# facebook/zstd

Hardware: NVIDIA H100
Metric: compress GB/s (input) at level 1 (higher is better)
Workload: dtype u8

## Files before the change

zstd_b200/csrc/zb_bitpack.cuh:

```cuda
#ifndef ZB_BITPACK_CUH
#define ZB_BITPACK_CUH
#include "zb_device.cuh"

struct ZbdParW { u32* words; u64 acc; u32 nacc; u32 widx; u32 first; };

__device__ __forceinline__ void zbd_pw_init(ZbdParW* w, u32* words, u64 bitPos)
{
    w->words = words; w->acc = 0; w->nacc = (u32)(bitPos & 31u); w->widx = (u32)(bitPos >> 5); w->first = 1;
}
__device__ __forceinline__ void zbd_pw_add(ZbdParW* w, u32 value, u32 nbBits)
{
    w->acc |= (u64)value << w->nacc;
    w->nacc += nbBits;
    if (w->nacc >= 32u) {
        u32 const lo = (u32)w->acc;
        if (w->first) { if (lo) atomicOr(&w->words[w->widx], lo); w->first = 0; }
        else w->words[w->widx] = lo;
        w->widx++;
        w->acc >>= 32;
        w->nacc -= 32u;
    }
}
__device__ __forceinline__ void zbd_pw_finish(ZbdParW* w)
{
    u32 const lo = (u32)w->acc;
    if (w->nacc && lo) atomicOr(&w->words[w->widx], lo);
}

#endif
```

zstd_b200/csrc/zb_entropy.cuh:

```cuda
#ifndef ZB_ENTROPY_CUH
#define ZB_ENTROPY_CUH
#include "zb_device.cuh"

#define ZBD_ERR 0xFFFFFFFFu

struct ZbdBitW { u8* out; u32 pos; u64 acc; u32 nacc; };
__device__ __forceinline__ void zbd_bw_init(ZbdBitW* w, u8* out) { w->out = out; w->pos = 0; w->acc = 0; w->nacc = 0; }
__device__ __forceinline__ void zbd_bw_add(ZbdBitW* w, u32 value, u32 nbBits)
{
    if (!nbBits) return;
    w->acc |= (u64)(value & ((1u << nbBits) - 1u)) << w->nacc;
    w->nacc += nbBits;
    while (w->nacc >= 8) { w->out[w->pos++] = (u8)w->acc; w->acc >>= 8; w->nacc -= 8; }
}
__device__ __forceinline__ u32 zbd_bw_close(ZbdBitW* w)
{
    zbd_bw_add(w, 1, 1);
    if (w->nacc) w->out[w->pos++] = (u8)w->acc;
    return w->pos;
}


__device__ __forceinline__ u32 zbd_fse_optimalTableLog(u32 maxTableLog, u32 srcSize, u32 maxSymbolValue, u32 minus)
{
    u32 const fromSource = zb_hb32(srcSize - 1u) - minus;
    u32 const needSrc = zb_hb32(srcSize) + 1u, needAlphabet = zb_hb32(maxSymbolValue) + 2u;
    u32 const floorLog = needSrc < needAlphabet ? needSrc : needAlphabet;
// ... 154 lines not shown

__device__ __forceinline__ u32 zbd_fse_initState2(const ZbdFseCTable* ct, u32 symbol)
{
    u32 const dnb = ct->deltaNbBits[symbol];
    u32 const nbBitsOut = (dnb + (1u << 15)) >> 16;
    u32 const value = (nbBitsOut << 16) - dnb;
    return ct->nextState[(int)(value >> nbBitsOut) + ct->deltaFindState[symbol]];
}
__device__ __forceinline__ u32 zbd_fse_step(const ZbdFseCTable* ct, u32 state, u32 symbol, u32* bits, u32* nb)
{
    u32 const nbBitsOut = (state + ct->deltaNbBits[symbol]) >> 16;
    *nb = nbBitsOut;
    *bits = state & ((1u << nbBitsOut) - 1u);
    return ct->nextState[(int)(state >> nbBitsOut) + ct->deltaFindState[symbol]];
}

struct ZbdHufWksp {
    u32 A[256];
    u16 rankSym[256];
    u8  len[256];
    u8  weights[256];
    u32 nl[16];
    u32 firstCode[16];
    u32 wcount[16];
    short wnorm[16];
    u8  symAt[64];
    u16 cum[66];
    u32 maxLen, nz;
    ZbdFseCTable wct;
};

template <int HUF_THREADS>
__device__ inline u32 zbc_huf_build(ZbdHufWksp* w, const u32* count, u32 maxSymbolValue, u32 target, u32* enc)
{
    u32 const tid = threadIdx.x;
    if (tid == 0) w->nz = 0;
    __syncthreads();
    {   u32 mine = 0;
        for (u32 s = tid; s < 256u; s += HUF_THREADS) {
            u32 const c = s <= maxSymbolValue ? count[s] : 0u;
            w->len[s] = 0;
            if (c) {
                u32 r = 0;
                for (u32 j = 0; j <= maxSymbolValue; j++) { u32 const cj = count[j]; r += (cj > c || (cj == c && j < s)) ? 1u : 0u; }
                w->rankSym[r] = (u16)s;
                mine++;
            }
        }
        if (mine) atomicAdd(&w->nz, mine);
    }
    __syncthreads();
    u32 const nz = w->nz;
    for (u32 i = tid; i < nz; i += HUF_THREADS) w->A[i] = count[w->rankSym[nz - 1u - i]];
    __syncthreads();
    if (tid == 0) {
        u32* const A = w->A;
        u32 root = 0, leaf = 2, next;
        A[0] += A[1];
        for (next = 1; next + 1u < nz; next++) {
            if (leaf >= nz || A[root] < A[leaf]) { A[next] = A[root]; A[root++] = next; } else A[next] = A[leaf++];
            if (leaf >= nz || (root < next && A[root] < A[leaf])) { A[next] += A[root]; A[root++] = next; } else A[next] += A[leaf++];
        }
        A[nz - 2u] = 0;
        for (next = nz - 2u; next-- > 0u; ) A[next] = A[A[next]] + 1u;
        {   int avbl = 1, used = 0, depth = 0;
            int rt = (int)nz - 2, nx = (int)nz - 1;
            while (avbl > 0) {
                while (rt >= 0 && (int)A[rt] == depth) { used++; rt--; }
                while (avbl > used) { A[nx--] = (u32)depth; avbl--; }
                avbl = 2 * used; depth++; used = 0;
            }
        }
        for (u32 l = 0; l < 16u; l++) w->nl[l] = 0;
    }
    __syncthreads();
    u32 const deepest = w->A[0];
// ... 6 lines not shown
            u32 K = 0;
            for (u32 l = target + 1u; l < 16u; l++) { nl[target] += nl[l]; nl[l] = 0; }
            for (u32 l = 1; l <= target; l++) K += nl[l] << (target - l);
            for (u32 E = K - (1u << target); E > 0u; E--) {
                u32 b = target - 1u;
                while (nl[b] == 0u) b--;
                nl[b]--; nl[b + 1u] += 2u; nl[target]--;
            }
            maxLen = target;
        }
        while (nl[maxLen] == 0u) maxLen--;
        w->maxLen = maxLen;
        u32 v = 0;
        for (u32 l = maxLen; l > 0u; l--) { w->firstCode[l] = v; v = (v + nl[l]) >> 1; }
    }
    __syncthreads();
    u32 const maxLen = w->maxLen;
    for (u32 r = tid; r < nz; r += HUF_THREADS) {
        u32 l = 1, acc = w->nl[1];
        while (r >= acc) { l++; acc += w->nl[l]; }
        w->len[w->rankSym[r]] = (u8)l;
    }
    __syncthreads();
    for (u32 s = tid; s < 256u; s += HUF_THREADS) {
        u32 const l = w->len[s];
        u32 e = 0;
        if (l) {
            u32 idx = 0;
            for (u32 j = 0; j < s; j++) idx += (w->len[j] == l) ? 1u : 0u;
            e = (w->firstCode[l] + idx) | (l << 16);
        }
        enc[s] = e;
    }
    __syncthreads();
    return maxLen;
}

template <int HUF_THREADS>
__device__ inline u32 zbc_huf_writeHeader(ZbdHufWksp* w, u8* dst, const u32* enc, u32 maxSymbolValue, u32 huffLog, u32* sh_result)
{
    u32 const tid = threadIdx.x, lane = tid & 31u;
    u8* const wt = w->weights;
    u32 const wtSize = maxSymbolValue;
    if (tid < 16u) w->wcount[tid] = 0;
    __syncthreads();
    for (u32 n = tid; n < wtSize; n += HUF_THREADS) {
        u32 const nb = enc[n] >> 16;
        u32 const v = nb ? huffLog + 1u - nb : 0u;
        wt[n] = (u8)v;
        atomicAdd(&w->wcount[v], 1u);
    }
    if (tid == 0) wt[wtSize] = 0;
    __syncthreads();
    if (tid < 32u) {
        u32 hSize = 0;
// ... 59 lines not shown
```

zstd_b200/csrc/zb_literals.cu:

```cuda
#include "zb_entropy.cuh"
#include "zb_kernels.h"

#define LIT_THREADS 128
#ifndef LIT_MIN_CTAS
#define LIT_MIN_CTAS 12
#endif
#define LIT_WARPS (LIT_THREADS / 32)
#define LIT_WIN 256u

__device__ void zb_hist256(const u8* __restrict__ src, u32 n, u32 (*whist)[256], u32* count)
{
    u32 const tid = threadIdx.x, warp = tid >> 5, lane = tid & 31u;
    for (u32 i = tid; i < LIT_WARPS * 256; i += LIT_THREADS) (&whist[0][0])[i] = 0;
    __syncthreads();
    u32 const head = (u32)((uintptr_t)src & 15u);
    const uint4* const v4 = reinterpret_cast<const uint4*>(src - head);
    u32 const seg = (n + 3u) / 4u;
    u32 const beg = min(warp * seg, n) + head, end = min((warp + 1u) * seg, n) + head;
    if (beg < end) {
        u32 const vLo = beg >> 4, nVec = ((end - 1u) >> 4) - vLo + 1u;
        uint4 nx = lane < nVec ? __ldg(v4 + vLo + lane) : make_uint4(0, 0, 0, 0);
        for (u32 i = lane; i < nVec; i += 32u) {
            uint4 const q = nx;
            if (i + 32u < nVec) nx = __ldg(v4 + vLo + i + 32u);
            u32 const p0 = (vLo + i) << 4;
            u32 const kLo = beg > p0 ? beg - p0 : 0u, kHi = min(end - p0, 16u);
            u32 const w[4] = { q.x, q.y, q.z, q.w };
#pragma unroll
            for (u32 k = 0; k < 16u; k++)
                if (k >= kLo && k < kHi) atomicAdd(&whist[warp][(w[k >> 2] >> (8u * (k & 3u))) & 0xFFu], 1u);
        }
    }
    __syncthreads();
    for (u32 sym = tid; sym < 256u; sym += LIT_THREADS) {
        u32 s = 0;
#pragma unroll
        for (int w = 0; w < LIT_WARPS; w++) s += whist[w][sym];
        count[sym] = s;
    }
    __syncthreads();
}

__device__ void zb_hist_stats(const u32* count, u32* red, u32* largestOut, u32* maxSymOut)
{
    u32 const tid = threadIdx.x;
    u32 c = 0, key = 0;
    for (u32 sym = tid; sym < 256u; sym += LIT_THREADS) { u32 const v = count[sym]; c = max(c, v); key = max(key, v ? sym : 0u); }
#pragma unroll
    for (int o = 16; o > 0; o >>= 1) {
        c = max(c, __shfl_xor_sync(ZB_FULL, c, o));
        key = max(key, __shfl_xor_sync(ZB_FULL, key, o));
    }
    if ((tid & 31) == 0) { red[tid >> 5] = c; red[8 + (tid >> 5)] = key; }
    __syncthreads();
    if (tid == 0) {
        u32 l = 0, m = 0;
        for (int w = 0; w < LIT_WARPS; w++) { l = max(l, red[w]); m = max(m, red[8 + w]); }
        *largestOut = l; *maxSymOut = m;
    }
    __syncthreads();
}

__device__ __forceinline__ void zb_huf_stream(const u8* __restrict__ lit, u32 beg, u32 end, const u32* enc, u32* win, u32* ow,
                                              u32 bitPos, u32 lane)
{
    const uint4* const v4 = reinterpret_cast<const uint4*>(lit);
    uint4 const zero = make_uint4(0, 0, 0, 0);
    u32 const vHi = (end - 1u) >> 4, nVec = vHi - (beg >> 4) + 1u;
    u32 const firstW = bitPos >> 5;
    uint4 q1 = lane < nVec ? __ldg(v4 + vHi - lane) : zero;
    uint4 q2 = lane + 32u < nVec ? __ldg(v4 + vHi - lane - 32u) : zero;
    for (u32 t = 0; t < nVec; t += 32u) {
        uint4 const q = q1;
        q1 = q2;
        q2 = t + 64u + lane < nVec ? __ldg(v4 + vHi - (t + 64u + lane)) : zero;
        u32 kLo = 0, kHi = 0;
        if (t + lane < nVec) { u32 const p0 = (vHi - t - lane) << 4; kLo = beg > p0 ? beg - p0 : 0u; kHi = min(end - p0, 16u); }
        u32 const w[4] = { q.x, q.y, q.z, q.w };
        u32 nb = 0;
#pragma unroll
        for (u32 k = 0; k < 16u; k++) {
            u32 const e = enc[(w[k >> 2] >> (8u * (k & 3u))) & 0xFFu];
            nb += (k >= kLo && k < kHi) ? e >> 16 : 0u;
        }
        u32 incl = nb;
#pragma unroll
        for (u32 o = 1; o < 32u; o <<= 1) { u32 const x = __shfl_up_sync(ZB_FULL, incl, o); if (lane >= o) incl += x; }
        u32 const tileBits = __shfl_sync(ZB_FULL, incl, 31);
        {
            u32 const p = bitPos + incl - nb;
            u32 widx = p >> 5, nacc = p & 31u, first = 1;
            u64 acc = 0;
#pragma unroll
            for (int k = 15; k >= 0; k--) {
                u32 const e = ((u32)k >= kLo && (u32)k < kHi) ? enc[(w[k >> 2] >> (8u * (k & 3u))) & 0xFFu] : 0u;
                acc |= (u64)(e & 0xFFFFu) << nacc;
                nacc += e >> 16;
                if (k & 1) continue;
                bool const full = nacc >= 32u;
                u32* const wp = win + widx % LIT_WIN;
                if (full && first == 0u) *wp = (u32)acc;
                if (full && first != 0u) atomicOr(wp, (u32)acc);
                first = full ? 0u : first;
                widx += full ? 1u : 0u;
                acc = full ? (acc >> 32) : acc;
                nacc -= full ? 32u : 0u;
            }
            if (nacc != 0u && (u32)acc != 0u) atomicOr(win + widx % LIT_WIN, (u32)acc);
        }
        __syncwarp();
        u32 const wEnd = (bitPos + tileBits) >> 5;
        for (u32 k = (bitPos >> 5) + lane; k < wEnd; k += 32u) {
            u32 const v = win[k % LIT_WIN];
            win[k % LIT_WIN] = 0u;
            if (k == firstW) atomicOr(ow + k, v); else ow[k] = v;
        }
        __syncwarp();
        bitPos += tileBits;
    }
    if (lane == 0) atomicOr(ow + (bitPos >> 5), win[(bitPos >> 5) % LIT_WIN] | (1u << (bitPos & 31u)));
}

__global__ void __launch_bounds__(LIT_THREADS, LIT_MIN_CTAS)
zb_literals_kernel(const ZbBlock* __restrict__ blocks, ZbParams prm, ZbStrides sd, const ZbDictEntropy* __restrict__ de,
                   const u8* __restrict__ lits, u8* __restrict__ body, ZbBlockMeta* __restrict__ meta)
{
    __shared__ __align__(16) u32 whist[LIT_WARPS][256];
    __shared__ ZbdHufWksp wk;
    __shared__ u32 count[256];
    __shared__ u32 enc[256];
    __shared__ __align__(16) u8 hdr[288];
    __shared__ u32 red[16];
    __shared__ u32 sh_largest, sh_maxSym, sh_mode, sh_hSize, sh_usePrev;
    __shared__ u32 sh_bits[LIT_WARPS];

    u32 const tid = threadIdx.x, warp = tid >> 5, lane = tid & 31u;
    u32 const b = blockIdx.x;
    ZbBlockMeta const m = meta[b];
    if (m.forceRaw) return;
    u32 const n = m.litSize;
    const u8* const lit = lits + (size_t)b * sd.lit;
    u8* const out = body + (size_t)b * sd.body;
    enum { MODE_RAW = 0, MODE_RLE = 1, MODE_HUF = 2 };

    u32 repeat = (de != nullptr && (blocks[b].flags & ZB_FLAG_FIRST) && de->present) ? de->hufRepeat : 0u;
    bool const preferRepeat = (n <= 1024u);
    u32 const lhSize = 3u + (n >= 1024u) + (n >= 16384u);
    u32 const nbStreams = (n < 256u || (repeat == 2u && lhSize == 3u)) ? 1u : 4u;
    u32 mode = MODE_HUF;
    bool usePrev = false;
    if (prm.litDisabled || n < (repeat == 2u ? 6u : 64u)) mode = MODE_RAW;
    if (mode == MODE_HUF && preferRepeat && repeat == 2u) usePrev = true;
    if (mode == MODE_HUF && !usePrev) {
        bool const suspect = (m.nbSeq == 0) || (n / m.nbSeq >= 20u);
        if (suspect && n >= 4096u * 10u) {
            u32 l1, l2;
            zb_hist256(lit, 4096u, whist, count);
            zb_hist_stats(count, red, &sh_largest, &sh_maxSym);
            l1 = sh_largest;
            __syncthreads();
            zb_hist256(lit + n - 4096u, 4096u, whist, count);
            zb_hist_stats(count, red, &sh_largest, &sh_maxSym);
            l2 = sh_largest;
            __syncthreads();
            if (l1 + l2 <= ((2u * 4096u) >> 7) + 4u) mode = MODE_RAW;
        }
    }
    if (mode == MODE_HUF) zb_hist256(lit, n, whist, count);
    if (mode == MODE_HUF && !usePrev) {
        zb_hist_stats(count, red, &sh_largest, &sh_maxSym);
        u32 const largest = sh_largest;
        if (largest == n) mode = MODE_RLE;
        else if (largest <= (n >> 7) + 4u) mode = MODE_RAW;
    }
    if (mode == MODE_HUF && !usePrev && repeat == 1u) {
        int bad = 0;
        for (u32 sym = tid; sym < 256u; sym += LIT_THREADS) bad |= (sym <= sh_maxSym) && count[sym] != 0u && (de->hufEnc[sym] >> 16) == 0u;
        if (__syncthreads_or(bad) || de->hufMaxSymbol < sh_maxSym) repeat = 0u;
    }
    if (mode == MODE_HUF && !usePrev && preferRepeat && repeat != 0u) usePrev = true;
    if (mode == MODE_HUF && !usePrev) {
        u32 const maxSym = sh_maxSym;
        u32 const huffLog = zbd_fse_optimalTableLog(11, n, maxSym, 1);
        u32 const maxBits = zbc_huf_build<LIT_THREADS>(&wk, count, maxSym, huffLog, enc);
        u32 const hSizeNew = (maxBits == ZBD_ERR) ? ZBD_ERR : zbc_huf_writeHeader<LIT_THREADS>(&wk, hdr, enc, maxSym, maxBits, &sh_hSize);
        if (tid == 0) {
            u32 md = MODE_HUF, hSize = 0, prev = 0;
            if (hSizeNew == ZBD_ERR) md = MODE_RAW;
            else {
                hSize = hSizeNew;
                if (repeat != 0u) {
                    u32 oldBits = 0, newBits = 0;
                    for (u32 sy = 0; sy <= maxSym; sy++) { oldBits += (de->hufEnc[sy] >> 16) * count[sy]; newBits += (enc[sy] >> 16) * count[sy]; }
                    if ((oldBits >> 3) <= hSize + (newBits >> 3) || hSize + 12u >= n) prev = 1;
                }
                if (!prev && hSize + 12u >= n) md = MODE_RAW;
            }
            sh_mode = md; sh_hSize = hSize; sh_usePrev = prev;
        }
        __syncthreads();
        mode = sh_mode;
        usePrev = sh_usePrev != 0u;
    }
    if (mode == MODE_HUF && usePrev) {
        __syncthreads();
        for (u32 sym = tid; sym < 256u; sym += LIT_THREADS) enc[sym] = de->hufEnc[sym];
        if (tid == 0) sh_hSize = 0;
        __syncthreads();
    }

    u32 const hType = usePrev ? 3u : 2u;
    u32 const seg = (n + 3u) / 4u;
    u32 streamSize[4] = { 0u, 0u, 0u, 0u };
    u32 hSize = 0, total = 0;
    if (mode == MODE_HUF) {
        hSize = sh_hSize;
        u32 bits = 0;
        for (u32 sym = lane; sym < 256u; sym += 32u) bits += whist[warp][sym] * (enc[sym] >> 16);
#pragma unroll
        for (int o = 16; o > 0; o >>= 1) bits += __shfl_xor_sync(ZB_FULL, bits, o);
        if (lane == 0) sh_bits[warp] = bits;
        __syncthreads();
        if (nbStreams == 4u) for (u32 k = 0; k < 4u; k++) streamSize[k] = (sh_bits[k] + 1u + 7u) >> 3;
        else streamSize[0] = (sh_bits[0] + sh_bits[1] + sh_bits[2] + sh_bits[3] + 1u + 7u) >> 3;
        u32 cSize = 0; bool tooBig = false;
#pragma unroll
        for (u32 k = 0; k < 4u; k++) { cSize += streamSize[k]; tooBig |= (streamSize[k] > 65535u); }
        if (nbStreams == 4u) cSize += 6u;
        total = hSize + cSize;
        if (nbStreams == 4u && tooBig) mode = MODE_RAW;
        else if (total >= n - 1u) mode = MODE_RAW;
        else if (total >= n - ((n >> 6) + 2u)) mode = MODE_RAW;
        else if (total == 1u) {
            int diff = 0;
            if (n < 8u) for (u32 i = tid; i < n; i += LIT_THREADS) diff |= (lit[i] != lit[0]);
            if (!__syncthreads_or(diff)) mode = MODE_RLE;
        }
    }

    if (mode == MODE_RAW) {
        u32 const flSize = 1u + (n > 31u) + (n > 4095u);
        if (tid == 0) {
            if (flSize == 1) out[0] = (u8)(0u + (n << 3));
            else if (flSize == 2) { u32 const v = 0u + (1u << 2) + (n << 4); out[0] = (u8)v; out[1] = (u8)(v >> 8); }
            else { u32 const v = 0u + (3u << 2) + (n << 4); out[0] = (u8)v; out[1] = (u8)(v >> 8); out[2] = (u8)(v >> 16); }
            meta[b].litSecSize = flSize + n;
        }
        for (u32 i = tid; i < n; i += LIT_THREADS) out[flSize + i] = lit[i];
        return;
    }
    if (mode == MODE_RLE) {
        if (tid == 0) {
            u32 const flSize = 1u + (n > 31u) + (n > 4095u);
            if (flSize == 1) out[0] = (u8)(1u + (n << 3));
            else if (flSize == 2) { u32 const v = 1u + (1u << 2) + (n << 4); out[0] = (u8)v; out[1] = (u8)(v >> 8); }
            else { u32 const v = 1u + (3u << 2) + (n << 4); out[0] = (u8)v; out[1] = (u8)(v >> 8); out[2] = (u8)(v >> 16); }
            out[flSize] = lit[0];
            meta[b].litSecSize = flSize + 1u;
        }
        return;
    }

    u32 sOff = lhSize + hSize + (nbStreams == 4u ? 6u : 0u), sSize = 0;
#pragma unroll
    for (u32 k = 0; k < 4u; k++) { sOff += k < warp ? streamSize[k] : 0u; sSize = k == warp ? streamSize[k] : sSize; }
    u32* const ow = reinterpret_cast<u32*>(out);
    for (u32 i = tid; i < LIT_WARPS * 256u; i += LIT_THREADS) (&whist[0][0])[i] = 0u;
    if (warp < nbStreams && lane == 0) { ow[sOff >> 2] = 0u; ow[(sOff + sSize - 1u) >> 2] = 0u; }
    __syncthreads();
    if (tid == 0) {
        u32 const cLitSize = total;
        if (lhSize == 3) { u32 const lhc = hType + ((nbStreams == 4u ? 1u : 0u) << 2) + (n << 4) + (cLitSize << 14);
                           out[0] = (u8)lhc; out[1] = (u8)(lhc >> 8); out[2] = (u8)(lhc >> 16); }
        else if (lhSize == 4) { u32 const lhc = hType + (2u << 2) + (n << 4) + (cLitSize << 18);
                           out[0] = (u8)lhc; out[1] = (u8)(lhc >> 8); out[2] = (u8)(lhc >> 16); out[3] = (u8)(lhc >> 24); }
        else { u32 const lhc = hType + (3u << 2) + (n << 4) + (cLitSize << 22);
                           out[0] = (u8)lhc; out[1] = (u8)(lhc >> 8); out[2] = (u8)(lhc >> 16); out[3] = (u8)(lhc >> 24);
                           out[4] = (u8)(cLitSize >> 10); }
        if (nbStreams == 4u) {
            u8* jt = out + lhSize + hSize;
            for (int k = 0; k < 3; k++) { jt[2 * k] = (u8)streamSize[k]; jt[2 * k + 1] = (u8)(streamSize[k] >> 8); }
        }
        meta[b].litSecSize = lhSize + total;
    }
    for (u32 i = tid; i < hSize; i += LIT_THREADS) out[lhSize + i] = hdr[i];
    __syncthreads();
    if (warp < nbStreams) {
        u32 const beg = nbStreams == 1u ? 0u : min(warp * seg, n), end = nbStreams == 1u ? n : min((warp + 1u) * seg, n);
        zb_huf_stream(lit, beg, end, enc, whist[warp], ow, sOff * 8u, lane);
    }
}

extern "C" cudaError_t zb_launch_literals(const ZbBlock* d_blocks, u32 nbBlocks, const ZbParams* prm, const ZbStrides* sd, const ZbDictEntropy* d_de,
                                          const u8* d_lits, u8* d_body, ZbBlockMeta* d_meta, cudaStream_t stream)
{
    if (nbBlocks == 0) return cudaSuccess;
    zb_literals_kernel<<<nbBlocks, LIT_THREADS, 0, stream>>>(d_blocks, *prm, *sd, d_de, d_lits, d_body, d_meta);
    return cudaGetLastError();
}
```

zstd_b200/csrc/zb_sequences.cu:

```cuda
#include "zb_entropy.cuh"
#include "zb_kernels.h"
#include "zb_bitpack.cuh"

#define SEQ_THREADS 128
#ifndef SEQ_TILE
#define SEQ_TILE 512u
#endif
#define MaxLL 35
#define MaxML 52
#define MaxOff 31
#define DefaultMaxOff 28
#define LLFSELog 9
#define MLFSELog 9
#define OffFSELog 8

__constant__ short c_LL_defaultNorm[MaxLL + 1] = { 4,3,2,2,2,2,2,2, 2,2,2,2,2,1,1,1, 2,2,2,2,2,2,2,2, 2,3,2,1,1,1,1,1, -1,-1,-1,-1 };
__constant__ short c_ML_defaultNorm[MaxML + 1] = { 1,4,3,2,2,2,2,2, 2,1,1,1,1,1,1,1, 1,1,1,1,1,1,1,1, 1,1,1,1,1,1,1,1,
                                                   1,1,1,1,1,1,1,1, 1,1,1,1,1,1,-1,-1, -1,-1,-1,-1,-1 };
__constant__ short c_OF_defaultNorm[DefaultMaxOff + 1] = { 1,1,1,1,1,1,2,2, 2,1,1,1,1,1,1,1, 1,1,1,1,1,1,1,1, -1,-1,-1,-1,-1 };

__device__ __forceinline__ u32 zbd_ll_code(u32 ll)
{
    if (ll > 63u) return zb_hb32(ll) + 19u;
    if (ll < 16u) return ll;
    if (ll < 24u) return 16u + ((ll - 16u) >> 1);
    if (ll < 32u) return 20u + ((ll - 24u) >> 2);
    if (ll < 48u) return 22u + ((ll - 32u) >> 3);
    return 24u;
}
__device__ __forceinline__ u32 zbd_ml_code(u32 mlBase)
// ... 33 lines not shown
    return s;
}

enum { set_basic = 0, set_rle = 1, set_compressed = 2, set_repeat = 3 };

__device__ __forceinline__ u32 zbd_selectEncodingType(u32 mostFrequent, u32 nbSeq, u32 defaultNormLog, bool defaultAllowed, u32 strategy, u32 prevRepeat)
{
    if (mostFrequent == nbSeq) return (defaultAllowed && nbSeq <= 2u) ? set_basic : set_rle;
    if (defaultAllowed) {
        u32 const mult = 10u - strategy;
        u32 const dynamicFse_nbSeq_min = ((1u << defaultNormLog) * mult) >> 3;
        if (prevRepeat == 2u && nbSeq < 1000u) return set_repeat;
        if (nbSeq < dynamicFse_nbSeq_min || mostFrequent < (nbSeq >> (defaultNormLog - 1u))) return set_basic;
    }
    return set_compressed;
}

__device__ ZbdFseCTable g_defaultCT[3];
extern "C" cudaError_t zb_upload_default_tables(const ZbdFseCTable* host3, cudaStream_t stream)
{
    return cudaMemcpyToSymbolAsync(g_defaultCT, host3, 3 * sizeof(ZbdFseCTable), 0, cudaMemcpyHostToDevice, stream);
}

struct ZbdStreamWork {
    u32 count[64];
    short norm[64];
    u8  nc[136];
    u8  symAt[512];
    u16 cum[66];
    u32 ncSize;
    u32 type;
    u32 finalState;
    u32 err;
};

__global__ void __launch_bounds__(SEQ_THREADS)
zb_sequences_kernel(const u8* __restrict__ src, const ZbBlock* __restrict__ blocks, ZbParams prm, ZbStrides sd, const ZbDictEntropy* __restrict__ de,
                    const u64* __restrict__ seqs, u16* __restrict__ stateBits,
                    u8* __restrict__ body, ZbBlockMeta* __restrict__ meta)
{
    __shared__ ZbdFseCTable ct[3];
    __shared__ ZbdStreamWork wk[3];
    __shared__ u32 chunkBits[SEQ_THREADS];
    __shared__ u32 stepTile[3][SEQ_TILE + 3u];
    __shared__ u32 sh_cSize, sh_hdrEnd, sh_streamSize;
    __shared__ ZbdCodeLut lut;

    u32 const tid = threadIdx.x;
    u32 const b = blockIdx.x;
    ZbBlockMeta const m = meta[b];
    ZbBlock const bd = blocks[b];
    if (m.forceRaw) return;
    u32 const nbSeq = m.nbSeq;
    const u64* const myseq = seqs + (size_t)b * sd.seq;
    u16* const myst = stateBits + (size_t)b * sd.dist;
    u8* const out = body + (size_t)b * sd.body;
    u32 op = m.litSecSize;

    u32 const nbSeqHdr = nbSeq < 128u ? 1u : (nbSeq < 0x7F00u ? 2u : 3u);
    if (tid == 0) {
        if (nbSeq < 128u) out[op] = (u8)nbSeq;
        else if (nbSeq < 0x7F00u) { out[op] = (u8)((nbSeq >> 8) + 0x80u); out[op + 1] = (u8)nbSeq; }
        else { out[op] = 0xFF; out[op + 1] = (u8)(nbSeq - 0x7F00u); out[op + 2] = (u8)((nbSeq - 0x7F00u) >> 8); }
    }
    op += nbSeqHdr;
    u32 cSize;
    if (nbSeq == 0) {
        cSize = op;
    } else {
        for (u32 i = tid; i < 192u; i += SEQ_THREADS) wk[i >> 6].count[i & 63u] = 0;
        for (u32 i = tid; i < 192u; i += SEQ_THREADS) { if (i < 64u) lut.ll[i] = (u16)zbd_ll_lut_entry(i); else lut.ml[i - 64u] = (u16)zbd_ml_lut_entry(i - 64u); }
        __syncthreads();
        for (u32 i = tid; i < nbSeq; i += SEQ_THREADS) {
            ZbdSeq const s = zbd_unpack(myseq[i], lut);
            atomicAdd(&wk[0].count[s.llc], 1u);
            atomicAdd(&wk[1].count[s.ofc], 1u);
            atomicAdd(&wk[2].count[s.mlc], 1u);
        }
        __syncthreads();
        if (tid < 96u) {
            u32 const st = tid >> 5, lane = tid & 31u;
            ZbdStreamWork* const w = &wk[st];
            u32 const maxAll = st == 0 ? MaxLL : (st == 1 ? MaxOff : MaxML);
            u32 const c0 = w->count[lane], c1 = (lane + 32u <= maxAll) ? w->count[lane + 32u] : 0u;
            u32 const hiUsed = __ballot_sync(ZB_FULL, c1 != 0u), loUsed = __ballot_sync(ZB_FULL, c0 != 0u);
            u32 const max = hiUsed ? 63u - (u32)__clz((int)hiUsed) : 31u - (u32)__clz((int)loUsed);
            u32 mostFrequent = c0 > c1 ? c0 : c1;
#pragma unroll
            for (u32 o = 16; o > 0; o >>= 1) mostFrequent = ::max(mostFrequent, __shfl_xor_sync(ZB_FULL, mostFrequent, o));
            u32 const defLog = st == 1 ? 5u : 6u;
            bool const defAllowed = st == 1 ? (max <= DefaultMaxOff) : true;
            u32 const prevRepeat = (de != nullptr && (bd.flags & ZB_FLAG_FIRST) && de->present) ? de->fseRepeat[st] : 0u;
            u32 const type = zbd_selectEncodingType(mostFrequent, nbSeq, defLog, defAllowed, prm.strategy, prevRepeat);
            if (lane == 0) { w->type = type; w->err = 0; w->ncSize = 0; }
            __syncwarp();
            if (type == set_repeat || type == set_basic) {
                const u32* from = reinterpret_cast<const u32*>(type == set_repeat ? &de->fse[st] : &g_defaultCT[st]);
                u32* to = reinterpret_cast<u32*>(&ct[st]);
                for (u32 i = lane; i < sizeof(ZbdFseCTable) / 4u; i += 32u) to[i] = from[i];
            } else if (type == set_rle) {
                if (lane == 0) {
                    ZbdSeq const first = zbd_unpack(myseq[0], lut);
// ... 2 lines not shown
                    w->nc[0] = (u8)sym; w->ncSize = 1;
                }
            } else {
                u32 const FSELog = st == 1 ? OffFSELog : (st == 0 ? LLFSELog : MLFSELog);
                u32 nbSeq_1 = nbSeq;
                u32 const tableLog = zbd_fse_optimalTableLog(FSELog, nbSeq, max, 2);
                {
                    ZbdSeq const last = zbd_unpack(myseq[nbSeq - 1], lut);
                    u32 const lastCode = st == 0 ? last.llc : (st == 1 ? last.ofc : last.mlc);
                    if (w->count[lastCode] > 1u) { nbSeq_1--; __syncwarp(); if (lane == 0) w->count[lastCode]--; }
                    __syncwarp();
                }
                u32 const r = zbw_fse_normalize(w->norm, tableLog, w->count, nbSeq_1, max, lane);
                u32 ncs = 0;
                if (r != ZBD_ERR) { if (lane == 0) ncs = zbd_fse_writeNCount(w->nc, w->norm, max, tableLog); ncs = __shfl_sync(ZB_FULL, ncs, 0); }
                if (r == ZBD_ERR || ncs == ZBD_ERR) { if (lane == 0) w->err = 1; }
                else {
                    if (lane == 0) w->ncSize = ncs;
                    zbw_fse_buildCTable(&ct[st], w->norm, max, tableLog, w->symAt, w->cum, lane);
                }
            }
        }
        __syncthreads();
        bool const err = wk[0].err | wk[1].err | wk[2].err;
        if (err) { if (tid == 0) { meta[b].type = ZB_BT_RAW; meta[b].bodySize = bd.size; } return; }

        {
            u32 state = 0;
            bool const chain = tid < 3u;
            u32 const st = chain ? tid : 0u;
            const u16* const ns = ct[st].nextState;
            const u32* const tw = stepTile[st] + 1;
            u16* const rec = myst + (size_t)st * sd.state;
            u32 const nbTiles = (nbSeq + SEQ_TILE - 1u) / SEQ_TILE;
            for (u32 tile = nbTiles; tile-- > 0; ) {
                u32 const t0 = tile * SEQ_TILE, t1 = min(t0 + SEQ_TILE, nbSeq);
                for (u32 i = t0 + tid; i < t1; i += SEQ_THREADS) {
                    ZbdSeq const s = zbd_unpack(myseq[i], lut);
                    stepTile[0][i - t0 + 1u] = ct[0].deltaNbBits[s.llc] | ((u32)ct[0].deltaFindState[s.llc] << 20);
                    stepTile[1][i - t0 + 1u] = ct[1].deltaNbBits[s.ofc] | ((u32)ct[1].deltaFindState[s.ofc] << 20);
                    stepTile[2][i - t0 + 1u] = ct[2].deltaNbBits[s.mlc] | ((u32)ct[2].deltaFindState[s.mlc] << 20);
                }
                __syncthreads();
                if (chain) {
                    u32 cnt = t1 - t0;
                    const u32* pw = tw + cnt;
                    u16* pr = rec + t1;
                    if (t1 == nbSeq) {
                        u32 const w0 = pw[-1], dnb = w0 & 0xFFFFFu;
                        u32 const nbOut = (dnb + (1u << 15)) >> 16;
                        state = ns[(int)(((nbOut << 16) - dnb) >> nbOut) + ((int)w0 >> 20)];
                        cnt--; pw--; pr--;
                    }
                    u32 w = pw[-1];
                    while (cnt) {
                        cnt--; pw--; pr--;
                        u32 const wn = pw[-1];
                        u32 const nb = (state + (w & 0xFFFFFu)) >> 16;
                        *pr = (u16)((state & ((1u << nb) - 1u)) | (nb << 12));
                        state = ns[(int)(state >> nb) + ((int)w >> 20)];
                        w = wn;
                    }
                }
                __syncthreads();
            }
            if (chain) wk[st].finalState = state;
        }
        __syncthreads();

        u32 const ncTotal = wk[0].ncSize + wk[1].ncSize + wk[2].ncSize;
        u32 const hdrEnd = op + 1u + ncTotal;
        u32 lastCountSize = 0;
        if (wk[0].type == set_compressed) lastCountSize = wk[0].ncSize;
        if (wk[1].type == set_compressed) lastCountSize = wk[1].ncSize;
        if (wk[2].type == set_compressed) lastCountSize = wk[2].ncSize;

        u32 const cs = (nbSeq + SEQ_THREADS - 1u) / SEQ_THREADS;
        u32 const cBeg = min(tid * cs, nbSeq), cEnd = min((tid + 1u) * cs, nbSeq);
        u32 bits = 0;
        for (u32 i = cBeg; i < cEnd; i++) {
            ZbdSeq const s = zbd_unpack(myseq[i], lut);
            bits += s.llBits + s.mlBits + s.ofc;
            if (i + 1u < nbSeq) bits += (myst[i] >> 12) + (myst[sd.state + i] >> 12) + (myst[2u * sd.state + i] >> 12);
        }
        chunkBits[tid] = bits;
        __syncthreads();
        u32 bitOff = 0;
        for (u32 k = tid + 1u; k < SEQ_THREADS; k++) bitOff += chunkBits[k];
        if (tid == 0) {
            u32 const totalBits = bitOff + bits + ct[2].tableLog + ct[1].tableLog + ct[0].tableLog + 1u;
            sh_streamSize = (totalBits + 7u) >> 3;
        }
        __syncthreads();
        u32 const streamSize = sh_streamSize;
        cSize = hdrEnd + streamSize;
        bool const fits = (cSize + 16u <= sd.body);
        if (fits) {
            u32 const w0 = hdrEnd >> 2, w1 = (cSize + 3u) >> 2;
            u32* const ow = reinterpret_cast<u32*>(out);
            for (u32 i = w0 + 1u + tid; i < w1; i += SEQ_THREADS) ow[i] = 0;
            if (tid == 0) {
                for (u32 i = hdrEnd; i < min((w0 + 1u) << 2, cSize + 4u); i++) out[i] = 0;
                u8* p = out + op;
                *p++ = (u8)((wk[0].type << 6) + (wk[1].type << 4) + (wk[2].type << 2));
                for (u32 st = 0; st < 3; st++) for (u32 i = 0; i < wk[st].ncSize; i++) *p++ = wk[st].nc[i];
            }
            __syncthreads();
            ZbdParW pw; zbd_pw_init(&pw, ow, (u64)hdrEnd * 8u + bitOff);
            for (u32 i = cEnd; i-- > cBeg; ) {
                ZbdSeq const s = zbd_unpack(myseq[i], lut);
                if (i + 1u < nbSeq) {
                    u32 const rOF = myst[sd.state + i], rML = myst[2u * sd.state + i], rLL = myst[i];
                    zbd_pw_add(&pw, rOF & 0xFFFu, rOF >> 12);
                    zbd_pw_add(&pw, rML & 0xFFFu, rML >> 12);
                    zbd_pw_add(&pw, rLL & 0xFFFu, rLL >> 12);
                }
                u32 const llb = s.llBits, mlb = s.mlBits;
                zbd_pw_add(&pw, s.litLen & ((1u << llb) - 1u), llb);
                zbd_pw_add(&pw, s.mlBase & ((1u << mlb) - 1u), mlb);
                zbd_pw_add(&pw, s.offBase & ((1u << s.ofc) - 1u), s.ofc);
            }
            if (tid == 0) {
                zbd_pw_add(&pw, wk[2].finalState & ((1u << ct[2].tableLog) - 1u), ct[2].tableLog);
                zbd_pw_add(&pw, wk[1].finalState & ((1u << ct[1].tableLog) - 1u), ct[1].tableLog);
                zbd_pw_add(&pw, wk[0].finalState & ((1u << ct[0].tableLog) - 1u), ct[0].tableLog);
                zbd_pw_add(&pw, 1u, 1u);
            }
            zbd_pw_finish(&pw);
        }
        if (!fits || (lastCountSize && (lastCountSize + streamSize) < 4u)) cSize = 0;
    }

    {   u32 const maxCSize = bd.size - ((bd.size >> 6) + 2u);
        if (cSize >= maxCSize) cSize = 0;
    }
    bool rle = false;
    if (!(bd.flags & ZB_FLAG_FIRST) && cSize < 25u) {
        const u8* const bsrc = src + bd.srcOff;
        u8 const v0 = bsrc[0];
        int diff = 0;
        for (u32 i = tid; i < bd.size; i += SEQ_THREADS) diff |= (bsrc[i] != v0);
        rle = !__syncthreads_or(diff);
    }
    if (tid == 0) {
        ZbBlockMeta mm = m;
        if (rle) { mm.type = ZB_BT_RLE; mm.bodySize = 1; mm.rleByte = src[bd.srcOff]; }
        else if (cSize == 0) { mm.type = ZB_BT_RAW; mm.bodySize = bd.size; }
        else { mm.type = ZB_BT_COMPRESSED; mm.bodySize = cSize; }
        meta[b] = mm;
    }
}

extern "C" cudaError_t zb_launch_sequences(const u8* d_src, const ZbBlock* d_blocks, u32 nbBlocks, const ZbParams* prm, const ZbStrides* sd, const ZbDictEntropy* d_de,
                                           const u64* d_seqs, u16* d_stateBits, u8* d_body, ZbBlockMeta* d_meta, cudaStream_t stream)
{
    if (nbBlocks == 0) return cudaSuccess;
    zb_sequences_kernel<<<nbBlocks, SEQ_THREADS, 0, stream>>>(d_src, d_blocks, *prm, *sd, d_de, d_seqs, d_stateBits, d_body, d_meta);
    return cudaGetLastError();
}
```

Baseline: 103.6.

## Parallelize Huffman build and sequence bitstream packing with warp scans and shared windows

Replaces the O(n^2) rank computation in Huffman table build with a block-wide bitonic sort, and the per-symbol code-index loop with warp ballots. The sequence bitstream writer changes from a per-thread chunked two-pass count-then-pack into a tiled warp-scan packer that stages words in a shared window (reusing the step tiles) before coalesced global stores. Literal Huffman encoding switches to a packed 16-bit code table and defers the first-word atomicOr, and the histogram gets a fast path for full 16-byte vectors. Optional clock instrumentation is added behind a compile flag. The tiled packer adds two block barriers per 128 sequences, which may cost more than the old single pass on short blocks.

New measurement: 104.8, median of 6. 1.1% higher.

```diff
diff --git a/zstd_b200/csrc/zb_bitpack.cuh b/zstd_b200/csrc/zb_bitpack.cuh
--- a/zstd_b200/csrc/zb_bitpack.cuh
+++ /dev/null
@@ -1,30 +0,0 @@
-#ifndef ZB_BITPACK_CUH
-#define ZB_BITPACK_CUH
-#include "zb_device.cuh"
-
-struct ZbdParW { u32* words; u64 acc; u32 nacc; u32 widx; u32 first; };
-
-__device__ __forceinline__ void zbd_pw_init(ZbdParW* w, u32* words, u64 bitPos)
-{
-    w->words = words; w->acc = 0; w->nacc = (u32)(bitPos & 31u); w->widx = (u32)(bitPos >> 5); w->first = 1;
-}
-__device__ __forceinline__ void zbd_pw_add(ZbdParW* w, u32 value, u32 nbBits)
-{
-    w->acc |= (u64)value << w->nacc;
-    w->nacc += nbBits;
-    if (w->nacc >= 32u) {
-        u32 const lo = (u32)w->acc;
-        if (w->first) { if (lo) atomicOr(&w->words[w->widx], lo); w->first = 0; }
-        else w->words[w->widx] = lo;
-        w->widx++;
-        w->acc >>= 32;
-        w->nacc -= 32u;
-    }
-}
-__device__ __forceinline__ void zbd_pw_finish(ZbdParW* w)
-{
-    u32 const lo = (u32)w->acc;
-    if (w->nacc && lo) atomicOr(&w->words[w->widx], lo);
-}
-
-#endif
diff --git a/zstd_b200/csrc/zb_entropy.cuh b/zstd_b200/csrc/zb_entropy.cuh
--- a/zstd_b200/csrc/zb_entropy.cuh
+++ b/zstd_b200/csrc/zb_entropy.cuh
@@ -3,6 +3,24 @@
 #include "zb_device.cuh"
 
 #define ZBD_ERR 0xFFFFFFFFu
+
+#ifdef ZB_ENTROPY_CLOCKS
+#define ZB_CLK_BEGIN(clk) u64 zbClk_ = clock64(); if (threadIdx.x == 0) atomicAdd(&(clk)[0], 1ull)
+#define ZB_CLK(clk, k) do { if (threadIdx.x == 0) { u64 const t_ = clock64(); atomicAdd(&(clk)[k], t_ - zbClk_); zbClk_ = t_; } } while (0)
+#define ZB_CLK_SYNC(clk, k) do { __syncthreads(); ZB_CLK(clk, k); } while (0)
+#define ZB_CLK_EXPORT(clk, name) \
+    extern "C" __attribute__((visibility("default"))) int name(unsigned long long* out, int n, int reset) \
+    {                                                                                                      \
+        if (cudaDeviceSynchronize() != cudaSuccess) return -1;                                             \
+        if (out && cudaMemcpyFromSymbol(out, clk, (size_t)n * 8u) != cudaSuccess) return -1;               \
+        if (reset) { unsigned long long z[16] = {}; if (cudaMemcpyToSymbol(clk, z, sizeof(clk)) != cudaSuccess) return -1; } \
+        return 0;                                                                                          \
+    }
+#else
+#define ZB_CLK_BEGIN(clk) do {} while (0)
+#define ZB_CLK(clk, k) do {} while (0)
+#define ZB_CLK_SYNC(clk, k) do {} while (0)
+#endif
 
 struct ZbdBitW { u8* out; u32 pos; u64 acc; u32 nacc; };
 __device__ __forceinline__ void zbd_bw_init(ZbdBitW* w, u8* out) { w->out = out; w->pos = 0; w->acc = 0; w->nacc = 0; }
@@ -203,36 +221,42 @@
     u8  weights[256];
     u32 nl[16];
     u32 firstCode[16];
+    u32 lenWarp[4][16];
     u32 wcount[16];
     short wnorm[16];
     u8  symAt[64];
     u16 cum[66];
-    u32 maxLen, nz;
+    u32 maxLen;
     ZbdFseCTable wct;
 };
 
 template <int HUF_THREADS>
 __device__ inline u32 zbc_huf_build(ZbdHufWksp* w, const u32* count, u32 maxSymbolValue, u32 target, u32* enc)
 {
-    u32 const tid = threadIdx.x;
-    if (tid == 0) w->nz = 0;
-    __syncthreads();
-    {   u32 mine = 0;
-        for (u32 s = tid; s < 256u; s += HUF_THREADS) {
-            u32 const c = s <= maxSymbolValue ? count[s] : 0u;
-            w->len[s] = 0;
-            if (c) {
-                u32 r = 0;
-                for (u32 j = 0; j <= maxSymbolValue; j++) { u32 const cj = count[j]; r += (cj > c || (cj == c && j < s)) ? 1u : 0u; }
-                w->rankSym[r] = (u16)s;
-                mine++;
-            }
-        }
-        if (mine) atomicAdd(&w->nz, mine);
-    }
-    __syncthreads();
-    u32 const nz = w->nz;
-    for (u32 i = tid; i < nz; i += HUF_THREADS) w->A[i] = count[w->rankSym[nz - 1u - i]];
+    static_assert(HUF_THREADS == 128, "two symbols per thread");
+    u32 const tid = threadIdx.x, lane = tid & 31u, warp = tid >> 5;
+    u32 nz;
+    {   u32 const c0 = tid <= maxSymbolValue ? count[tid] : 0u, c1 = tid + 128u <= maxSymbolValue ? count[tid + 128u] : 0u;
+        w->A[tid] = c0 ? (c0 << 8) | (255u - tid) : 0u;
+        w->A[tid + 128u] = c1 ? (c1 << 8) | (127u - tid) : 0u;
+        w->len[tid] = 0; w->len[tid + 128u] = 0;
+        nz = __syncthreads_count(c0 != 0u) + __syncthreads_count(c1 != 0u);
+    }
+    for (u32 k = 2u; k <= 256u; k <<= 1) {
+        for (u32 j = k >> 1; j > 0u; j >>= 1) {
+            u32 const i = (tid / j) * 2u * j + (tid % j);
+            u32 const a = w->A[i], b = w->A[i + j];
+            if (((i & k) == 0u) == (a < b)) { w->A[i] = b; w->A[i + j] = a; }
+            __syncthreads();
+        }
+    }
+    {   u32 const k0 = w->A[tid], k1 = w->A[tid + 128u];
+        if (tid < nz) w->rankSym[tid] = (u16)(255u - (k0 & 0xFFu));
+        if (tid + 128u < nz) w->rankSym[tid + 128u] = (u16)(255u - (k1 & 0xFFu));
+        __syncthreads();
+        if (tid < nz) w->A[nz - 1u - tid] = k0 >> 8;
+        if (tid + 128u < nz) w->A[nz - 129u - tid] = k1 >> 8;
+    }
     __syncthreads();
     if (tid == 0) {
         u32* const A = w->A;
@@ -285,15 +309,19 @@
         w->len[w->rankSym[r]] = (u8)l;
     }
     __syncthreads();
-    for (u32 s = tid; s < 256u; s += HUF_THREADS) {
-        u32 const l = w->len[s];
-        u32 e = 0;
-        if (l) {
-            u32 idx = 0;
-            for (u32 j = 0; j < s; j++) idx += (w->len[j] == l) ? 1u : 0u;
-            e = (w->firstCode[l] + idx) | (l << 16);
-        }
-        enc[s] = e;
+    {   u32 const s0 = 2u * tid, l0 = w->len[s0], l1 = w->len[s0 + 1u], below = (1u << lane) - 1u;
+        u32 i0 = 0, i1 = 0;
+        for (u32 l = 1; l <= maxLen; l++) {
+            u32 const b0 = __ballot_sync(ZB_FULL, l0 == l), b1 = __ballot_sync(ZB_FULL, l1 == l);
+            u32 const before = (u32)__popc(b0 & below) + (u32)__popc(b1 & below);
+            i0 = l0 == l ? before : i0;
+            i1 = l1 == l ? before + (l0 == l ? 1u : 0u) : i1;
+            if (lane == 0) w->lenWarp[warp][l] = (u32)__popc(b0) + (u32)__popc(b1);
+        }
+        __syncthreads();
+        for (u32 v = 0; v < warp; v++) { i0 += l0 ? w->lenWarp[v][l0] : 0u; i1 += l1 ? w->lenWarp[v][l1] : 0u; }
+        enc[s0] = l0 ? (w->firstCode[l0] + i0) | (l0 << 16) : 0u;
+        enc[s0 + 1u] = l1 ? (w->firstCode[l1] + i1) | (l1 << 16) : 0u;
     }
     __syncthreads();
     return maxLen;
diff --git a/zstd_b200/csrc/zb_literals.cu b/zstd_b200/csrc/zb_literals.cu
--- a/zstd_b200/csrc/zb_literals.cu
+++ b/zstd_b200/csrc/zb_literals.cu
@@ -8,9 +8,15 @@
 #define LIT_WARPS (LIT_THREADS / 32)
 #define LIT_WIN 256u
 
+#ifdef ZB_ENTROPY_CLOCKS
+__device__ unsigned long long g_zbLitClk[16];
+ZB_CLK_EXPORT(g_zbLitClk, ZSTDB200_literalsClocks)
+#endif
+
 __device__ void zb_hist256(const u8* __restrict__ src, u32 n, u32 (*whist)[256], u32* count)
 {
     u32 const tid = threadIdx.x, warp = tid >> 5, lane = tid & 31u;
+    u32* const bins = whist[warp];
     for (u32 i = tid; i < LIT_WARPS * 256; i += LIT_THREADS) (&whist[0][0])[i] = 0;
     __syncthreads();
     u32 const head = (u32)((uintptr_t)src & 15u);
@@ -26,9 +32,14 @@
             u32 const p0 = (vLo + i) << 4;
             u32 const kLo = beg > p0 ? beg - p0 : 0u, kHi = min(end - p0, 16u);
             u32 const w[4] = { q.x, q.y, q.z, q.w };
-#pragma unroll
-            for (u32 k = 0; k < 16u; k++)
-                if (k >= kLo && k < kHi) atomicAdd(&whist[warp][(w[k >> 2] >> (8u * (k & 3u))) & 0xFFu], 1u);
+            if (kLo == 0u && kHi == 16u) {
+#pragma unroll
+                for (u32 k = 0; k < 16u; k++) atomicAdd(&bins[(w[k >> 2] >> (8u * (k & 3u))) & 0xFFu], 1u);
+            } else {
+#pragma unroll
+                for (u32 k = 0; k < 16u; k++)
+                    if (k >= kLo && k < kHi) atomicAdd(&bins[(w[k >> 2] >> (8u * (k & 3u))) & 0xFFu], 1u);
+            }
         }
     }
     __syncthreads();
@@ -61,7 +72,7 @@
     __syncthreads();
 }
 
-__device__ __forceinline__ void zb_huf_stream(const u8* __restrict__ lit, u32 beg, u32 end, const u32* enc, u32* win, u32* ow,
+__device__ __forceinline__ void zb_huf_stream(const u8* __restrict__ lit, u32 beg, u32 end, const u16* enc, u32* win, u32* ow,
                                               u32 bitPos, u32 lane)
 {
     const uint4* const v4 = reinterpret_cast<const uint4*>(lit);
@@ -77,11 +88,14 @@
         u32 kLo = 0, kHi = 0;
         if (t + lane < nVec) { u32 const p0 = (vHi - t - lane) << 4; kLo = beg > p0 ? beg - p0 : 0u; kHi = min(end - p0, 16u); }
         u32 const w[4] = { q.x, q.y, q.z, q.w };
+        u32 e2[8];
         u32 nb = 0;
 #pragma unroll
-        for (u32 k = 0; k < 16u; k++) {
-            u32 const e = enc[(w[k >> 2] >> (8u * (k & 3u))) & 0xFFu];
-            nb += (k >= kLo && k < kHi) ? e >> 16 : 0u;
+        for (u32 k = 0; k < 16u; k += 2u) {
+            u32 const a = (k >= kLo && k < kHi) ? (u32)enc[(w[k >> 2] >> (8u * (k & 3u))) & 0xFFu] : 0u;
+            u32 const c = (k + 1u >= kLo && k + 1u < kHi) ? (u32)enc[(w[k >> 2] >> (8u * ((k + 1u) & 3u))) & 0xFFu] : 0u;
+            e2[k >> 1] = a | (c << 16);
+            nb += (a >> 12) + (c >> 12);
         }
         u32 incl = nb;
 #pragma unroll
@@ -89,23 +103,24 @@
         u32 const tileBits = __shfl_sync(ZB_FULL, incl, 31);
         {
             u32 const p = bitPos + incl - nb;
-            u32 widx = p >> 5, nacc = p & 31u, first = 1;
+            u32 const w0 = p >> 5;
+            u32 widx = w0, nacc = p & 31u, first = 1, firstWord = 0;
             u64 acc = 0;
 #pragma unroll
             for (int k = 15; k >= 0; k--) {
-                u32 const e = ((u32)k >= kLo && (u32)k < kHi) ? enc[(w[k >> 2] >> (8u * (k & 3u))) & 0xFFu] : 0u;
-                acc |= (u64)(e & 0xFFFFu) << nacc;
-                nacc += e >> 16;
+                u32 const e = (k & 1) ? e2[k >> 1] >> 16 : e2[k >> 1] & 0xFFFFu;
+                acc |= (u64)(e & 0xFFFu) << nacc;
+                nacc += e >> 12;
                 if (k & 1) continue;
                 bool const full = nacc >= 32u;
-                u32* const wp = win + widx % LIT_WIN;
-                if (full && first == 0u) *wp = (u32)acc;
-                if (full && first != 0u) atomicOr(wp, (u32)acc);
+                if (full && first == 0u) win[widx % LIT_WIN] = (u32)acc;
+                firstWord = (full && first != 0u) ? (u32)acc : firstWord;
                 first = full ? 0u : first;
                 widx += full ? 1u : 0u;
                 acc = full ? (acc >> 32) : acc;
                 nacc -= full ? 32u : 0u;
             }
+            if (firstWord != 0u) atomicOr(win + w0 % LIT_WIN, firstWord);
             if (nacc != 0u && (u32)acc != 0u) atomicOr(win + widx % LIT_WIN, (u32)acc);
         }
         __syncwarp();
@@ -129,6 +144,7 @@
     __shared__ ZbdHufWksp wk;
     __shared__ u32 count[256];
     __shared__ u32 enc[256];
+    __shared__ u16 enc16[256];
     __shared__ __align__(16) u8 hdr[288];
     __shared__ u32 red[16];
     __shared__ u32 sh_largest, sh_maxSym, sh_mode, sh_hSize, sh_usePrev;
@@ -138,6 +154,7 @@
     u32 const b = blockIdx.x;
     ZbBlockMeta const m = meta[b];
     if (m.forceRaw) return;
+    ZB_CLK_BEGIN(g_zbLitClk);
     u32 const n = m.litSize;
     const u8* const lit = lits + (size_t)b * sd.lit;
     u8* const out = body + (size_t)b * sd.body;
@@ -166,7 +183,9 @@
             if (l1 + l2 <= ((2u * 4096u) >> 7) + 4u) mode = MODE_RAW;
         }
     }
+    ZB_CLK(g_zbLitClk, 1);
     if (mode == MODE_HUF) zb_hist256(lit, n, whist, count);
+    ZB_CLK(g_zbLitClk, 2);
     if (mode == MODE_HUF && !usePrev) {
         zb_hist_stats(count, red, &sh_largest, &sh_maxSym);
         u32 const largest = sh_largest;
@@ -179,10 +198,12 @@
         if (__syncthreads_or(bad) || de->hufMaxSymbol < sh_maxSym) repeat = 0u;
     }
     if (mode == MODE_HUF && !usePrev && preferRepeat && repeat != 0u) usePrev = true;
+    ZB_CLK(g_zbLitClk, 3);
     if (mode == MODE_HUF && !usePrev) {
         u32 const maxSym = sh_maxSym;
         u32 const huffLog = zbd_fse_optimalTableLog(11, n, maxSym, 1);
         u32 const maxBits = zbc_huf_build<LIT_THREADS>(&wk, count, maxSym, huffLog, enc);
+        ZB_CLK(g_zbLitClk, 4);
         u32 const hSizeNew = (maxBits == ZBD_ERR) ? ZBD_ERR : zbc_huf_writeHeader<LIT_THREADS>(&wk, hdr, enc, maxSym, maxBits, &sh_hSize);
         if (tid == 0) {
             u32 md = MODE_HUF, hSize = 0, prev = 0;
@@ -208,6 +229,7 @@
         if (tid == 0) sh_hSize = 0;
         __syncthreads();
     }
+    ZB_CLK(g_zbLitClk, 5);
 
     u32 const hType = usePrev ? 3u : 2u;
     u32 const seg = (n + 3u) / 4u;
@@ -237,6 +259,7 @@
             if (!__syncthreads_or(diff)) mode = MODE_RLE;
         }
     }
+    ZB_CLK(g_zbLitClk, 6);
 
     if (mode == MODE_RAW) {
         u32 const flSize = 1u + (n > 31u) + (n > 4095u);
@@ -247,6 +270,7 @@
             meta[b].litSecSize = flSize + n;
         }
         for (u32 i = tid; i < n; i += LIT_THREADS) out[flSize + i] = lit[i];
+        ZB_CLK_SYNC(g_zbLitClk, 7);
         return;
     }
     if (mode == MODE_RLE) {
@@ -258,6 +282,7 @@
             out[flSize] = lit[0];
             meta[b].litSecSize = flSize + 1u;
         }
+        ZB_CLK_SYNC(g_zbLitClk, 7);
         return;
     }
 
@@ -265,7 +290,8 @@
 #pragma unroll
     for (u32 k = 0; k < 4u; k++) { sOff += k < warp ? streamSize[k] : 0u; sSize = k == warp ? streamSize[k] : sSize; }
     u32* const ow = reinterpret_cast<u32*>(out);
-    for (u32 i = tid; i < LIT_WARPS * 256u; i += LIT_THREADS) (&whist[0][0])[i] = 0u;
+    for (u32 i = tid; i < LIT_WARPS * LIT_WIN; i += LIT_THREADS) (&whist[0][0])[i] = 0u;
+    for (u32 sym = tid; sym < 256u; sym += LIT_THREADS) enc16[sym] = (u16)((enc[sym] & 0xFFFu) | ((enc[sym] >> 16) << 12));
     if (warp < nbStreams && lane == 0) { ow[sOff >> 2] = 0u; ow[(sOff + sSize - 1u) >> 2] = 0u; }
     __syncthreads();
     if (tid == 0) {
@@ -287,8 +313,9 @@
     __syncthreads();
     if (warp < nbStreams) {
         u32 const beg = nbStreams == 1u ? 0u : min(warp * seg, n), end = nbStreams == 1u ? n : min((warp + 1u) * seg, n);
-        zb_huf_stream(lit, beg, end, enc, whist[warp], ow, sOff * 8u, lane);
-    }
+        zb_huf_stream(lit, beg, end, enc16, whist[warp], ow, sOff * 8u, lane);
+    }
+    ZB_CLK_SYNC(g_zbLitClk, 7);
 }
 
 extern "C" cudaError_t zb_launch_literals(const ZbBlock* d_blocks, u32 nbBlocks, const ZbParams* prm, const ZbStrides* sd, const ZbDictEntropy* d_de,
diff --git a/zstd_b200/csrc/zb_sequences.cu b/zstd_b200/csrc/zb_sequences.cu
--- a/zstd_b200/csrc/zb_sequences.cu
+++ b/zstd_b200/csrc/zb_sequences.cu
@@ -1,11 +1,11 @@
 #include "zb_entropy.cuh"
 #include "zb_kernels.h"
-#include "zb_bitpack.cuh"
 
 #define SEQ_THREADS 128
 #ifndef SEQ_TILE
 #define SEQ_TILE 512u
 #endif
+#define SEQ_WIN 1024u
 #define MaxLL 35
 #define MaxML 52
 #define MaxOff 31
@@ -85,6 +85,11 @@
     return cudaMemcpyToSymbolAsync(g_defaultCT, host3, 3 * sizeof(ZbdFseCTable), 0, cudaMemcpyHostToDevice, stream);
 }
 
+#ifdef ZB_ENTROPY_CLOCKS
+__device__ unsigned long long g_zbSeqClk[16];
+ZB_CLK_EXPORT(g_zbSeqClk, ZSTDB200_sequencesClocks)
+#endif
+
 struct ZbdStreamWork {
     u32 count[64];
     short norm[64];
@@ -104,16 +109,17 @@
 {
     __shared__ ZbdFseCTable ct[3];
     __shared__ ZbdStreamWork wk[3];
-    __shared__ u32 chunkBits[SEQ_THREADS];
+    __shared__ u32 warpBits[SEQ_THREADS / 32];
     __shared__ u32 stepTile[3][SEQ_TILE + 3u];
-    __shared__ u32 sh_cSize, sh_hdrEnd, sh_streamSize;
     __shared__ ZbdCodeLut lut;
+    static_assert(SEQ_WIN <= 3u * (SEQ_TILE + 3u), "the bit-stream window lives in the step tiles");
 
     u32 const tid = threadIdx.x;
     u32 const b = blockIdx.x;
     ZbBlockMeta const m = meta[b];
     ZbBlock const bd = blocks[b];
     if (m.forceRaw) return;
+    ZB_CLK_BEGIN(g_zbSeqClk);
     u32 const nbSeq = m.nbSeq;
     const u64* const myseq = seqs + (size_t)b * sd.seq;
     u16* const myst = stateBits + (size_t)b * sd.dist;
@@ -141,6 +147,7 @@
             atomicAdd(&wk[2].count[s.mlc], 1u);
         }
         __syncthreads();
+        ZB_CLK(g_zbSeqClk, 1);
         if (tid < 96u) {
             u32 const st = tid >> 5, lane = tid & 31u;
             ZbdStreamWork* const w = &wk[st];
@@ -189,6 +196,7 @@
             }
         }
         __syncthreads();
+        ZB_CLK(g_zbSeqClk, 2);
         bool const err = wk[0].err | wk[1].err | wk[2].err;
         if (err) { if (tid == 0) { meta[b].type = ZB_BT_RAW; meta[b].bodySize = bd.size; } return; }
 
@@ -234,6 +242,7 @@
             if (chain) wk[st].finalState = state;
         }
         __syncthreads();
+        ZB_CLK(g_zbSeqClk, 3);
 
         u32 const ncTotal = wk[0].ncSize + wk[1].ncSize + wk[2].ncSize;
         u32 const hdrEnd = op + 1u + ncTotal;
@@ -242,59 +251,84 @@
         if (wk[1].type == set_compressed) lastCountSize = wk[1].ncSize;
         if (wk[2].type == set_compressed) lastCountSize = wk[2].ncSize;
 
-        u32 const cs = (nbSeq + SEQ_THREADS - 1u) / SEQ_THREADS;
-        u32 const cBeg = min(tid * cs, nbSeq), cEnd = min((tid + 1u) * cs, nbSeq);
-        u32 bits = 0;
-        for (u32 i = cBeg; i < cEnd; i++) {
-            ZbdSeq const s = zbd_unpack(myseq[i], lut);
-            bits += s.llBits + s.mlBits + s.ofc;
-            if (i + 1u < nbSeq) bits += (myst[i] >> 12) + (myst[sd.state + i] >> 12) + (myst[2u * sd.state + i] >> 12);
-        }
-        chunkBits[tid] = bits;
-        __syncthreads();
-        u32 bitOff = 0;
-        for (u32 k = tid + 1u; k < SEQ_THREADS; k++) bitOff += chunkBits[k];
-        if (tid == 0) {
-            u32 const totalBits = bitOff + bits + ct[2].tableLog + ct[1].tableLog + ct[0].tableLog + 1u;
-            sh_streamSize = (totalBits + 7u) >> 3;
-        }
-        __syncthreads();
-        u32 const streamSize = sh_streamSize;
+        u32* const win = &stepTile[0][0];
+        u32* const ow = reinterpret_cast<u32*>(out);
+        u32 const wLim = sd.body >> 2, firstW = hdrEnd >> 2;
+        for (u32 i = tid; i < SEQ_WIN; i += SEQ_THREADS) win[i] = 0;
+        if (tid == 0 && hdrEnd + 4u <= sd.body) {
+            for (u32 i = hdrEnd; i < ((firstW + 1u) << 2); i++) out[i] = 0;
+            u8* p = out + op;
+            *p++ = (u8)((wk[0].type << 6) + (wk[1].type << 4) + (wk[2].type << 2));
+            for (u32 st = 0; st < 3; st++) for (u32 i = 0; i < wk[st].ncSize; i++) *p++ = wk[st].nc[i];
+        }
+        __syncthreads();
+        ZB_CLK(g_zbSeqClk, 4);
+        u32 const lane = tid & 31u, warp = tid >> 5;
+        u32 pos = hdrEnd * 8u;
+        for (u32 t0 = 0; t0 <= nbSeq; t0 += SEQ_THREADS) {
+            u32 f[6] = { 0u, 0u, 0u, 0u, 0u, 0u };
+            if (t0 + tid < nbSeq) {
+                u32 const i = nbSeq - 1u - t0 - tid;
+                ZbdSeq const sq = zbd_unpack(myseq[i], lut);
+                if (i + 1u < nbSeq) {
+                    u32 const rOF = myst[sd.state + i], rML = myst[2u * sd.state + i], rLL = myst[i];
+                    f[0] = ((rOF & 0xFFFu) << 5) | (rOF >> 12);
+                    f[1] = ((rML & 0xFFFu) << 5) | (rML >> 12);
+                    f[2] = ((rLL & 0xFFFu) << 5) | (rLL >> 12);
+                }
+                f[3] = ((sq.litLen & ((1u << sq.llBits) - 1u)) << 5) | sq.llBits;
+                f[4] = ((sq.mlBase & ((1u << sq.mlBits) - 1u)) << 5) | sq.mlBits;
+                f[5] = ((sq.offBase & ((1u << sq.ofc) - 1u)) << 5) | sq.ofc;
+            } else if (t0 + tid == nbSeq) {
+                f[0] = ((wk[2].finalState & ((1u << ct[2].tableLog) - 1u)) << 5) | ct[2].tableLog;
+                f[1] = ((wk[1].finalState & ((1u << ct[1].tableLog) - 1u)) << 5) | ct[1].tableLog;
+                f[2] = ((wk[0].finalState & ((1u << ct[0].tableLog) - 1u)) << 5) | ct[0].tableLog;
+                f[3] = (1u << 5) | 1u;
+            }
+            u32 nb = 0;
+#pragma unroll
+            for (u32 k = 0; k < 6u; k++) nb += f[k] & 31u;
+            u32 incl = nb;
+#pragma unroll
+            for (u32 o = 1; o < 32u; o <<= 1) { u32 const x = __shfl_up_sync(ZB_FULL, incl, o); if (lane >= o) incl += x; }
+            if (lane == 31u) warpBits[warp] = incl;
+            __syncthreads();
+            u32 below = 0, tileBits = 0;
+#pragma unroll
+            for (u32 v = 0; v < SEQ_THREADS / 32u; v++) { u32 const x = warpBits[v]; below += v < warp ? x : 0u; tileBits += x; }
+            {   u32 const p = pos + below + incl - nb;
+                u32 widx = p >> 5, nacc = p & 31u, first = 1;
+                u64 acc = 0;
+#pragma unroll
+                for (u32 k = 0; k < 6u; k++) {
+                    acc |= (u64)(f[k] >> 5) << nacc;
+                    nacc += f[k] & 31u;
+                    if (nacc >= 32u) {
+                        u32* const wp = win + widx % SEQ_WIN;
+                        if (first) atomicOr(wp, (u32)acc); else *wp = (u32)acc;
+                        first = 0; widx++; acc >>= 32; nacc -= 32u;
+                    }
+                }
+                if (nacc != 0u && (u32)acc != 0u) atomicOr(win + widx % SEQ_WIN, (u32)acc);
+            }
+            __syncthreads();
+            bool const last = t0 + SEQ_THREADS > nbSeq;
+            u32 const wEnd = (pos + tileBits + (last ? 31u : 0u)) >> 5;
+            u32 fw = 0;
+            for (u32 k = (pos >> 5) + tid; k < wEnd; k += SEQ_THREADS) {
+                u32 const v = win[k % SEQ_WIN];
+                win[k % SEQ_WIN] = 0u;
+                if (k != firstW && k < wLim) ow[k] = v;
+                fw = k == firstW ? v : fw;
+            }
+            if (fw != 0u && firstW < wLim) atomicOr(ow + firstW, fw);
+            __syncthreads();
+            pos += tileBits;
+        }
+        ZB_CLK(g_zbSeqClk, 5);
+        u32 const streamSize = (pos - hdrEnd * 8u + 7u) >> 3;
         cSize = hdrEnd + streamSize;
         bool const fits = (cSize + 16u <= sd.body);
-        if (fits) {
-            u32 const w0 = hdrEnd >> 2, w1 = (cSize + 3u) >> 2;
-            u32* const ow = reinterpret_cast<u32*>(out);
-            for (u32 i = w0 + 1u + tid; i < w1; i += SEQ_THREADS) ow[i] = 0;
-            if (tid == 0) {
-                for (u32 i = hdrEnd; i < min((w0 + 1u) << 2, cSize + 4u); i++) out[i] = 0;
-                u8* p = out + op;
-                *p++ = (u8)((wk[0].type << 6) + (wk[1].type << 4) + (wk[2].type << 2));
-                for (u32 st = 0; st < 3; st++) for (u32 i = 0; i < wk[st].ncSize; i++) *p++ = wk[st].nc[i];
-            }
-            __syncthreads();
-            ZbdParW pw; zbd_pw_init(&pw, ow, (u64)hdrEnd * 8u + bitOff);
-            for (u32 i = cEnd; i-- > cBeg; ) {
-                ZbdSeq const s = zbd_unpack(myseq[i], lut);
-                if (i + 1u < nbSeq) {
-                    u32 const rOF = myst[sd.state + i], rML = myst[2u * sd.state + i], rLL = myst[i];
-                    zbd_pw_add(&pw, rOF & 0xFFFu, rOF >> 12);
-                    zbd_pw_add(&pw, rML & 0xFFFu, rML >> 12);
-                    zbd_pw_add(&pw, rLL & 0xFFFu, rLL >> 12);
-                }
-                u32 const llb = s.llBits, mlb = s.mlBits;
-                zbd_pw_add(&pw, s.litLen & ((1u << llb) - 1u), llb);
-                zbd_pw_add(&pw, s.mlBase & ((1u << mlb) - 1u), mlb);
-                zbd_pw_add(&pw, s.offBase & ((1u << s.ofc) - 1u), s.ofc);
-            }
-            if (tid == 0) {
-                zbd_pw_add(&pw, wk[2].finalState & ((1u << ct[2].tableLog) - 1u), ct[2].tableLog);
-                zbd_pw_add(&pw, wk[1].finalState & ((1u << ct[1].tableLog) - 1u), ct[1].tableLog);
-                zbd_pw_add(&pw, wk[0].finalState & ((1u << ct[0].tableLog) - 1u), ct[0].tableLog);
-                zbd_pw_add(&pw, 1u, 1u);
-            }
-            zbd_pw_finish(&pw);
-        }
         if (!fits || (lastCountSize && (lastCountSize + streamSize) < 4u)) cSize = 0;
     }
 
@@ -316,6 +350,7 @@
         else { mm.type = ZB_BT_COMPRESSED; mm.bodySize = cSize; }
         meta[b] = mm;
     }
+    ZB_CLK_SYNC(g_zbSeqClk, 6);
 }
 
 extern "C" cudaError_t zb_launch_sequences(const u8* d_src, const ZbBlock* d_blocks, u32 nbBlocks, const ZbParams* prm, const ZbStrides* sd, const ZbDictEntropy* d_de,
```
